# MengRao/pollnet

Hardware: AMD Instinct MI355X
Metric: device-resident Gbit/s + Mframes/s, 1500 B IPv4/TCP frames, 1/2/4/8 MI355X (higher is better)
Workload: dtype u16/u32 integer (one's-complement sums)

## Files before the change

pollnet_amd/csrc/rx_service.hip:

```cpp
#include <algorithm>
#include <chrono>
#include <cstdlib>

#include "rx_classify.hpp"

namespace {
using pn_internal::hip_err;
using pn_internal::set_err;

struct alignas(64) SvcPost {
  uint32_t gen;
  uint32_t n;
  uint32_t fpw;
  uint32_t max_conn;
  const uint8_t* frames;
  pn_result* out;
  const pn_conn_entry* tbl;
  uint16_t* links;
  uint32_t mask;
  uint32_t n_entries;
  uint32_t check;
  uint32_t seq;
};
static_assert(sizeof(SvcPost) == 64, "one line per post");

constexpr uint32_t kDoneWords = 64;
constexpr uint32_t kCountWords = 64;
constexpr uint32_t kExitWord = 96;
constexpr uint32_t kWordsBytes = 512;
constexpr uint32_t kLatWaves = PN_SERVICE_WAVES;
static_assert(kLatWaves <= kDoneWords, "a latency-tier post completes through per-wave done words");
constexpr uint32_t kLatFrames = kLatWaves * kFramesPerWave;
constexpr uint32_t kNetLimitMs = 8000;
constexpr uint32_t kPostVerify = 1u << 30, kPostLinks = 1u << 29, kPostN = (1u << 21) - 1;
constexpr uint32_t kLinkFrames = PN_LINK_MAX_FRAMES, kLinkConns = PN_LINK_MAX_CONNS;
constexpr uint32_t kMailBytes = 4096;

struct alignas(64) SvcDev {
  uint32_t count[2][16];
};
constexpr uint32_t kExitFlag = 32;

#ifdef PN_SVC_TRACE
__device__ uint64_t* g_svc_trace = nullptr;
#define SVC_T(w, i)                                                       \
  do {                                                                    \
    if (lane == 0 && (w) < 64) g_svc_trace[(w) * 8 + (i)] = wall_clock64(); \
  } while (0)
#else
#define SVC_T(w, i) \
  do {              \
  } while (0)
#endif

struct SArgs {
  const SvcPost* mail;
  u32x4* scratch;
  uint32_t* done_words;
  uint32_t* exit_word;
  SvcDev* dev;
  uint64_t idle_ticks;
  uint64_t net_ticks;
  uint32_t epoch;
  uint32_t last;
  uint32_t stride, ipa_off, avail;
  uint32_t poll_sleep;
};

inline uint32_t svc_fpw(uint32_t n, bool verify) {
  uint32_t fpw = verify ? 8u : kFramesPerWave;
  while (fpw < kFramesPerWave && (n + fpw - 1) / fpw > kLatWaves) fpw <<= 1;
  return fpw;
}

inline uint32_t svc_check(const SvcPost* p, uint32_t k) {
  const uint32_t* w = reinterpret_cast<const uint32_t*>(p);
  uint32_t x = k;
  for (int i = 1; i <= 13; i++) x ^= w[i];
  return x;
}

__host__ __device__ __forceinline__ uint32_t svc_active(uint32_t n, uint32_t fpw, uint32_t waves) {
  const uint32_t groups = (n + fpw - 1) / fpw;
  return groups < waves ? groups : waves;
}

inline uint32_t svc_helpers(uint32_t n, uint32_t max) {
  if (n <= kLatFrames) return 0;
  const uint32_t groups = (n + kFramesPerWave - 1) / kFramesPerWave;
  return std::min(groups - kLatWaves, max);
}

__device__ __forceinline__ KArgsAux svc_args(uint32_t v, uint32_t b, const SArgs& s, uint32_t k) {
  auto w32 = [&](uint32_t i) { return (uint32_t)__builtin_amdgcn_readlane(v, b + i); };
  auto u64 = [&](uint32_t lo) { return ((uint64_t)w32(lo + 1) << 32) | w32(lo); };
  KArgsAux a;
  const uint32_t nw = w32(1);
  a.n = nw & kPostN;
  a.fpw = w32(2) & 0xffu;
  a.max_conn = w32(3);
  a.frames = reinterpret_cast<const uint8_t*>(u64(4));
  a.out = reinterpret_cast<pn_result*>(u64(6));
  a.tbl = reinterpret_cast<const pn_conn_entry*>(u64(8));
  a.mask = w32(12);
  a.n_entries = w32(13);
  a.stride = s.stride;
  a.ipa_off = s.ipa_off;
  a.avail = s.avail;
  a.offs = nullptr;
  a.aux = (nw & kPostLinks) ? s.scratch + (size_t)(k & 1) * kLinkFrames * 2 : nullptr;
  return a;
}

__device__ __forceinline__ uint16_t* svc_links(uint32_t v, uint32_t b) {
  return reinterpret_cast<uint16_t*>(((uint64_t)(uint32_t)__builtin_amdgcn_readlane(v, b + 11) << 32) |
                                     (uint32_t)__builtin_amdgcn_readlane(v, b + 10));
}

constexpr uint32_t kCleanNeed = PN_F_HIT | PN_F_ACK | PN_F_IP_OK;
constexpr uint32_t kCleanNone = PN_F_TW | PN_F_SYN | PN_F_FIN | PN_F_RST | PN_F_NOT_TCP | PN_F_TRUNC | PN_F_BADOFF |
                                PN_F_IHL_NE_5;

struct ChainLds {
  uint32_t last[kLinkConns];
  uint32_t key[kLinkFrames];
  uint32_t seq_end[kLinkFrames];
  u32x4 fields[kLinkFrames];
};

__device__ __forceinline__ ChainLds& chain_lds() {
  __shared__ ChainLds c;
  return c;
}

__device__ __forceinline__ void chain_init(int lane) {
  ChainLds& c = chain_lds();
  for (uint32_t i = lane; i < kLinkConns; i += kWave) c.last[i] = 0u;
  wave_lds_sync();
}

__device__ __forceinline__ void chain_step(ChainLds& c, uint32_t base, uint32_t n, uint32_t max_conn, bool on,
                                           const u32x4& rec, const u32x4& fx, const __amdgpu_buffer_rsrc_t& lr,
                                           uint64_t below, int lane) {
  const uint32_t i = base + lane;
  const bool valid = i < n;
  const uint32_t flags = rec.w & 0xffffu;
  const uint32_t len = rec.z >> 16;
  const bool member = on && valid && (flags & (PN_F_HIT | PN_F_TW)) == PN_F_HIT && rec.x < max_conn;
  const bool usable = (flags & kCleanNeed) == kCleanNeed && (flags & kCleanNone) == 0 &&
                      (flags & (PN_F_TCP_OK | PN_F_TCP_UNCHECKED)) != 0 && len != 0 && len < 0x8000u;
  const uint32_t key = member ? rec.x : 0u;
  if (valid) {
    c.key[i] = member ? key : 0xFFFFFFFFu;
    c.seq_end[i] = rec.y + len;
    c.fields[i] = u32x4{fx.x, fx.y, fx.z, (rec.z & 0xffffu) | (usable ? 0x10000u : 0u)};
  }
  uint32_t prev = 0;
  if (member) prev = c.last[key];
  wave_lds_sync();
  if (member) atomicMax(&c.last[key], i + 1);
  wave_lds_sync();
  uint64_t todo = __ballot(member && c.last[key] != i + 1);
  while (todo) {
    const uint32_t leader = (uint32_t)__builtin_ctzll(todo);
    const uint32_t kk = __builtin_amdgcn_readlane(key, leader);
    const uint64_t m = __ballot(member && key == kk);
    todo &= ~m;
    const uint64_t lower = m & below;
    if (member && key == kk && lower) prev = base + 64u - (uint32_t)__builtin_clzll(lower);
  }
  uint32_t d = 0;
  if (member && usable && prev) {
    const uint32_t j = prev - 1;
    const u32x4 pf = c.fields[j];
    if ((pf.w >> 16) && c.seq_end[j] == rec.y && pf.x == fx.x && pf.y == fx.y && pf.z == fx.z &&
        (pf.w & 0xffffu) == (rec.z & 0xffffu))
      d = i - j;
  }
  if (valid) __builtin_amdgcn_raw_buffer_store_b16((unsigned short)d, lr, i * 2, 0, 0);
  wave_lds_sync();
}

__device__ __forceinline__ void chain_pass(const u32x4* aux, uint32_t n, uint32_t max_conn, uint16_t* links, int lane) {
  constexpr int kChunk = 8;
  ChainLds& c = chain_lds();
  const bool on = max_conn <= kLinkConns;
  const __amdgpu_buffer_rsrc_t lr = frame_rsrc(reinterpret_cast<const uint8_t*>(links), n * 2);
  const __amdgpu_buffer_rsrc_t ar = frame_rsrc(reinterpret_cast<const uint8_t*>(aux), n * 32);
  const uint64_t below = (1ull << lane) - 1;
  for (uint32_t base0 = 0; base0 < n; base0 += kChunk * kWave) {
    u32x4 rec[kChunk], fx[kChunk];
#pragma unroll
    for (int s = 0; s < kChunk; ++s) {
      const uint32_t i = base0 + s * kWave + lane;
      rec[s] = __builtin_amdgcn_raw_buffer_load_b128(ar, i * 32, 0, 0);
      fx[s] = __builtin_amdgcn_raw_buffer_load_b128(ar, i * 32 + 16, 0, 0);
    }
#pragma unroll
    for (int s = 0; s < kChunk; ++s)
      if (base0 + s * kWave < n) chain_step(c, base0 + s * kWave, n, max_conn, on, rec[s], fx[s], lr, below, lane);
  }
  for (uint32_t i = lane; i < n; i += kWave) {
    const uint32_t k = c.key[i];
    if (k != 0xFFFFFFFFu) c.last[k] = 0u;
  }
  wave_lds_sync();
}

template <int MIS, int COOP, bool HELPER = false>
__device__ __forceinline__ void svc_run(const KArgsAux& a, bool verify, bool linked, uint32_t w, uint32_t act, uint32_t k,
                                        uint32_t* done_word, int lane) {
  for (uint32_t g = w; g * a.fpw < a.n; g += act) {
    if (verify) classify_group<MIS, COOP, kProdAbl | kChainAux, kLoadAux, kStoreAux, 0, kLoadAux>(a, g * a.fpw, lane);
    else
      classify_group<MIS, COOP, kProdAbl | kHeaderOnly | kChainAux, kLoadAux, kStoreAux, 0, kLoadAux>(a, g * a.fpw, lane);
  }
  if constexpr (HELPER) return;
  __threadfence_system();
  if (lane == 0 && act <= kDoneWords && !linked)
    __hip_atomic_store(done_word, k, __ATOMIC_RELAXED, __HIP_MEMORY_SCOPE_SYSTEM);
}

template <bool PASS>
__device__ __forceinline__ void svc_finish(const KArgsAux& a, uint16_t* links, uint32_t k, uint32_t* count_word, int lane) {
  if constexpr (PASS) {
    if (a.aux) {
      __builtin_amdgcn_fence(__ATOMIC_ACQUIRE, "agent");
      chain_pass(a.aux, a.n, a.max_conn, links, lane);
    }
  }
  __threadfence_system();
  if (lane == 0) __hip_atomic_store(count_word, k, __ATOMIC_RELAXED, __HIP_MEMORY_SCOPE_SYSTEM);
}

template <bool PASS>
__device__ __forceinline__ void svc_count(uint32_t* count, const KArgsAux& a, uint16_t* links, uint32_t target, uint32_t k,
                                          uint32_t* count_word, int lane) {
  uint32_t prev = 0;
  if (lane == 0) prev = atomicAdd(count, 1u);
  prev = __builtin_amdgcn_readfirstlane(prev);
  if (prev == target - 1) {
    if (lane == 0) __hip_atomic_store(count, 0u, __ATOMIC_RELAXED, __HIP_MEMORY_SCOPE_AGENT);
    svc_finish<PASS>(a, links, k, count_word, lane);
  }
}

template <int MIS, int COOP>
__global__ __launch_bounds__(kWave) void rx_service_kernel(SArgs s) {
  const int lane = threadIdx.x;
  const uint32_t w = blockIdx.x, W = gridDim.x;
  const uint32_t* mw = reinterpret_cast<const uint32_t*>(s.mail);
  uint32_t last = s.last;
  uint64_t t0 = wall_clock64();
  chain_init(lane);
  for (;;) {
    const uint32_t v = lane <= (int)kExitFlag ? __hip_atomic_load(mw + lane, __ATOMIC_RELAXED, __HIP_MEMORY_SCOPE_SYSTEM) : 0u;
    if (w != 0 && (uint32_t)__builtin_amdgcn_readlane(v, kExitFlag) == s.epoch) return;
    const uint32_t k = last + 1;
    const uint32_t b = (k & 1) * 16;
    const uint32_t q = __builtin_amdgcn_readlane(v, b + 15);
    uint32_t x = q;
#pragma unroll
    for (uint32_t i = 1; i <= 13; i++) x ^= (uint32_t)__builtin_amdgcn_readlane(v, b + i);
    const bool whole = (uint32_t)__builtin_amdgcn_readlane(v, b) == q && (uint32_t)__builtin_amdgcn_readlane(v, b + 14) == x;
    if (!whole || (int32_t)(q - k) < 0) {
      if (w == 0) {
        if (wall_clock64() - t0 > s.idle_ticks) {
          if (lane == 0) {
            __hip_atomic_store(const_cast<uint32_t*>(mw) + kExitFlag, s.epoch, __ATOMIC_RELAXED, __HIP_MEMORY_SCOPE_SYSTEM);
            __hip_atomic_store(s.exit_word, s.epoch, __ATOMIC_RELEASE, __HIP_MEMORY_SCOPE_SYSTEM);
          }
          return;
        }
        __builtin_amdgcn_s_sleep(1);
      } else {
        if (wall_clock64() - t0 > s.net_ticks) return;
        for (uint32_t i = 0; i < s.poll_sleep; ++i) __builtin_amdgcn_s_sleep(1);
      }
      continue;
    }
    if (q != k) {
      last = k;
      t0 = wall_clock64();
      continue;
    }
    const uint32_t nw = __builtin_amdgcn_readlane(v, b + 1);
    if (nw == PN_SERVICE_STOP) return;
    last = k;
    const uint32_t fw = __builtin_amdgcn_readlane(v, b + 2);
    const uint32_t act = svc_active(nw & kPostN, fw & 0xffu, W + (fw >> 8));
    if (w < act) {
      SVC_T(w, 0);
      __builtin_amdgcn_fence(__ATOMIC_ACQUIRE, "");
      SVC_T(w, 1);
      const KArgsAux a = svc_args(v, b, s, k);
      SVC_T(w, 5);
      const bool linked = a.aux != nullptr;
      svc_run<MIS, COOP>(a, (nw & kPostVerify) != 0, linked, w, act, k, s.done_words + w, lane);
      SVC_T(w, 6);
      if (act > kDoneWords || linked) {
        uint32_t* cw = s.done_words + kCountWords + (k & 1);
        if (act == 1) svc_finish<true>(a, svc_links(v, b), k, cw, lane);
        else svc_count<true>(&s.dev->count[k & 1][0], a, svc_links(v, b), act < W ? act : W, k, cw, lane);
      }
      SVC_T(w, 7);
    }
    t0 = wall_clock64();
  }
}

template <int MIS, int COOP>
__global__ __launch_bounds__(kWave) void rx_service_helper_kernel(KArgsAux a, uint32_t verify, uint32_t act) {
  svc_run<MIS, COOP, true>(a, verify != 0, false, kLatWaves + blockIdx.x, act, 0, nullptr, threadIdx.x);
}

template <int MIS>
void launch_svc(bool coop, uint32_t waves, const SArgs& a, hipStream_t s) {
  if (coop) hipLaunchKernelGGL((rx_service_kernel<MIS, 1>), dim3(waves), dim3(kWave), 0, s, a);
  else hipLaunchKernelGGL((rx_service_kernel<MIS, 0>), dim3(waves), dim3(kWave), 0, s, a);
}

template <int MIS>
void launch_helpers(bool coop, uint32_t helpers, const KArgsAux& a, uint32_t verify, uint32_t act, hipStream_t s) {
  if (coop) hipLaunchKernelGGL((rx_service_helper_kernel<MIS, 1>), dim3(helpers), dim3(kWave), 0, s, a, verify, act);
  else hipLaunchKernelGGL((rx_service_helper_kernel<MIS, 0>), dim3(helpers), dim3(kWave), 0, s, a, verify, act);
}
}

struct pn_service {
  pn_ctx* ctx = nullptr;
  hipStream_t stream = nullptr;
  hipStream_t helper_stream = nullptr;
  uint32_t stride = 0, frame_off = 0;
  uint32_t helpers_max = 0;
  uint32_t post_helpers[2] = {0, 0};
  hipEvent_t helper_ev[2] = {nullptr, nullptr};
  uint64_t idle_ticks = 0, net_ticks = 0;
  SvcPost* mail = nullptr;
  bool mail_dev = false;
  uint32_t* words = nullptr;
  uint32_t post_words[2] = {0, 0};
  uint32_t tbl_post[2] = {0, 0};
  bool tbl_used[2] = {false, false};
  SvcDev* dev = nullptr;
  u32x4* scratch = nullptr;
  uint32_t seq = 0;
  uint32_t epoch = 0;
  bool running = false;
  bool coop = false;
};

namespace {
SArgs svc_sargs(const pn_service* v, uint32_t base) {
  SArgs a;
  a.mail = v->mail;
  a.scratch = v->scratch;
  a.done_words = v->words;
  a.exit_word = v->words + kExitWord;
  a.dev = v->dev;
  a.idle_ticks = v->idle_ticks;
  a.net_ticks = v->net_ticks;
  a.epoch = v->epoch;
  a.last = base;
  a.stride = v->stride;
  a.ipa_off = (v->frame_off + 14) & ~15u;
  a.avail = v->stride - v->frame_off;
  a.poll_sleep = v->mail_dev ? 1u : 16u;
  return a;
}

inline void host_sfence() { asm volatile("sfence" ::: "memory"); }

void svc_publish(SvcPost* slot, const SvcPost& q, bool wc) {
  static const bool avx = __builtin_cpu_supports("avx");
  if (wc && avx) {
    asm volatile(
        "vmovdqu (%0), %%ymm0\n\t"
        "vmovdqu 32(%0), %%ymm1\n\t"
        "vmovntdq %%ymm0, (%1)\n\t"
        "vmovntdq %%ymm1, 32(%1)\n\t"
        "sfence\n\t"
        "vzeroupper"
        :
        : "r"(&q), "r"(slot)
        : "memory", "xmm0", "xmm1");
    return;
  }
  volatile uint32_t* d = reinterpret_cast<volatile uint32_t*>(slot);
  const uint32_t* w = reinterpret_cast<const uint32_t*>(&q);
  for (int i = 1; i <= 14; ++i) d[i] = w[i];
  host_sfence();
  d[0] = w[0];
  d[15] = w[15];
  host_sfence();
}

int svc_launch_helpers(pn_service* v, uint32_t k, uint32_t helpers, const SvcPost& q) {
  KArgsAux a;
  strided_kargs(a, q.frames, q.out, q.tbl, q.mask, q.n_entries, q.max_conn, q.n & kPostN, v->stride, v->frame_off);
  a.fpw = q.fpw & 0xffu;
  const uint32_t verify = (q.n & kPostVerify) ? 1u : 0u, act = svc_active(a.n, a.fpw, kLatWaves + helpers);
  hipStream_t s = v->helper_stream;
  for_mis(v->frame_off, [&](auto mis) { launch_helpers<mis()>(v->coop, helpers, a, verify, act, s); });
  hipError_t e = hipGetLastError();
  if (e == hipSuccess && !v->helper_ev[k & 1]) e = hipEventCreateWithFlags(&v->helper_ev[k & 1], hipEventDisableTiming);
  if (e == hipSuccess) e = hipEventRecord(v->helper_ev[k & 1], s);
  if (e != hipSuccess) return hip_err(v->ctx, e, "pn_service: helper launch");
  return PN_OK;
}

int svc_launch(pn_service* v, uint32_t base) {
  pn_ctx* ctx = v->ctx;
  const SvcDev init{};
  hipError_t e = hipMemcpyAsync(v->dev, &init, sizeof(SvcDev), hipMemcpyHostToDevice, v->stream);
  if (e == hipSuccess) e = hipStreamSynchronize(v->stream);
  if (e != hipSuccess) return hip_err(ctx, e, "pn_service: device state");
  if (++v->epoch == 0) ++v->epoch;
  const SArgs a = svc_sargs(v, base);
  for_mis(v->frame_off, [&](auto mis) { launch_svc<mis()>(v->coop, kLatWaves, a, v->stream); });
  e = hipGetLastError();
  if (e != hipSuccess) return hip_err(ctx, e, "pn_service: launch");
  v->running = true;
  return PN_OK;
}

bool svc_post_ran(const pn_service* v, uint32_t k) {
  const uint32_t words = v->post_words[k & 1];
  if (words == 0 && (int32_t)(__atomic_load_n(v->words + kCountWords + (k & 1), __ATOMIC_ACQUIRE) - k) < 0) return false;
  for (uint32_t w = 0; w < words; ++w)
    if ((int32_t)(__atomic_load_n(v->words + w, __ATOMIC_ACQUIRE) - k) < 0) return false;
  if (v->post_helpers[k & 1] && hipEventQuery(v->helper_ev[k & 1]) != hipSuccess) return false;
  return true;
}

bool svc_post_done(const pn_service* v, uint32_t k) {
  if ((int32_t)(v->seq - k) >= 2) return true;
  if (!svc_post_ran(v, k)) return false;
  return k != v->seq || svc_post_ran(v, k - 1);
}

uint32_t svc_done(const pn_service* v) {
  if (svc_post_done(v, v->seq)) return v->seq;
  return svc_post_done(v, v->seq - 1) ? v->seq - 1 : v->seq - 2;
}

bool svc_exited(const pn_service* v) { return __atomic_load_n(v->words + kExitWord, __ATOMIC_ACQUIRE) == v->epoch; }

void svc_free(pn_service* v) {
  if (v->ctx) {
    auto& l = v->ctx->services;
    l.erase(std::remove(l.begin(), l.end(), v), l.end());
  }
  if (v->mail) (void)(v->mail_dev ? hipFree(v->mail) : hipHostFree(v->mail));
  if (v->words) (void)hipHostFree(v->words);
  if (v->dev) (void)hipFree(v->dev);
  if (v->scratch) (void)hipFree(v->scratch);
  if (v->stream) (void)hipStreamDestroy(v->stream);
  if (v->helper_stream) (void)hipStreamDestroy(v->helper_stream);
  for (hipEvent_t ev : v->helper_ev)
    if (ev) (void)hipEventDestroy(ev);
  delete v;
}
}

int pn_internal::svc_release_table(pn_ctx* ctx, int buf) {
  for (pn_service* v : ctx->services) {
    if (!v->tbl_used[buf]) continue;
    const uint32_t id = v->tbl_post[buf];
    if ((int32_t)(v->seq - id) < 2 && !svc_post_done(v, id)) {
      const int rc = pn_service_wait(v, id);
      if (rc) return rc;
    }
    v->tbl_used[buf] = false;
  }
  return PN_OK;
}

extern "C" {

int pn_service_open(pn_ctx* ctx, uint32_t slot_stride, uint32_t frame_off, uint32_t idle_ms, pn_service** out) {
  return pn_service_open_ex(ctx, slot_stride, frame_off, idle_ms, 0, out);
}

int pn_service_open_ex(pn_ctx* ctx, uint32_t slot_stride, uint32_t frame_off, uint32_t idle_ms, uint32_t large_waves,
                       pn_service** out) {
  if (!ctx || !out) return set_err(ctx, PN_EINVAL, "pn_service_open: ctx / out is NULL");
  *out = nullptr;
  if ((slot_stride & 15) || slot_stride > 65536 || (frame_off & 1) || slot_stride < frame_off + 96)
    return set_err(ctx, PN_EINVAL, "pn_service_open: slot_stride/frame_off violate the layout contract");
  if (idle_ms == 0 || idle_ms > 10000) return set_err(ctx, PN_EINVAL, "pn_service_open: idle_ms must be in [1, 10000]");
  if (large_waves && (large_waves < PN_SERVICE_WAVES || large_waves > PN_SERVICE_MAX_WAVES))
    return set_err(ctx, PN_EINVAL, "pn_service_open: large_waves must be 0 or in [PN_SERVICE_WAVES, PN_SERVICE_MAX_WAVES]");
  hipError_t e = hipSetDevice(ctx->device);
  if (e != hipSuccess) return hip_err(ctx, e, "hipSetDevice");
  int khz = 0;
  e = hipDeviceGetAttribute(&khz, hipDeviceAttributeWallClockRate, ctx->device);
  if (e != hipSuccess || khz <= 0) return hip_err(ctx, e, "pn_service_open: wall clock rate");
  int cus = 0;
  e = hipDeviceGetAttribute(&cus, hipDeviceAttributeMultiprocessorCount, ctx->device);
  if (e != hipSuccess || cus <= 0) return hip_err(ctx, e, "pn_service_open: CU count");
  pn_service* v = new pn_service();
  v->ctx = ctx;
  v->stride = slot_stride;
  v->frame_off = frame_off;
  const uint32_t total = large_waves ? large_waves
                                     : std::max<uint32_t>(kLatWaves, std::min<uint32_t>(PN_SERVICE_MAX_WAVES,
                                                                                      (uint32_t)cus * PN_SERVICE_WAVES_PER_CU));
  v->helpers_max = total - kLatWaves;
  v->idle_ticks = (uint64_t)khz * idle_ms;
  v->net_ticks = v->idle_ticks + (v->idle_ticks >> 1) + (uint64_t)khz * kNetLimitMs;
  v->coop = (slot_stride % 16) == 0 && ((frame_off + 14) & ~15u) >= 16;
  int large_bar = 0;
  if (hipDeviceGetAttribute(&large_bar, hipDeviceAttributeIsLargeBar, ctx->device) != hipSuccess) large_bar = 0;
  v->mail_dev = large_bar != 0 && std::getenv("PN_SERVICE_HOST_MAILBOX") == nullptr;
  if (v->mail_dev && hipExtMallocWithFlags((void**)&v->mail, kMailBytes, hipDeviceMallocUncached) != hipSuccess) {
    (void)hipGetLastError();
    v->mail = nullptr;
    v->mail_dev = false;
  }
  if ((e = hipStreamCreateWithFlags(&v->stream, hipStreamNonBlocking)) != hipSuccess ||
      (e = hipStreamCreateWithFlags(&v->helper_stream, hipStreamNonBlocking)) != hipSuccess ||
      (!v->mail && (e = hipHostMalloc((void**)&v->mail, kMailBytes, hipHostMallocDefault)) != hipSuccess) ||
      (e = hipHostMalloc((void**)&v->words, kWordsBytes, hipHostMallocDefault)) != hipSuccess ||
      (e = hipMalloc((void**)&v->dev, sizeof(SvcDev))) != hipSuccess ||
      (e = hipMalloc((void**)&v->scratch, sizeof(u32x4) * 2 * 2 * kLinkFrames)) != hipSuccess) {
    const int rc = hip_err(ctx, e, "pn_service_open: allocation");
    svc_free(v);
    return rc;
  }
  uint32_t first = 0;
  if (const char* env = std::getenv("PN_SERVICE_FIRST_POST")) first = (uint32_t)std::strtoull(env, nullptr, 0);
  std::memset(v->words, 0, kWordsBytes);
  for (uint32_t w = 0; w < kDoneWords + 2; ++w) v->words[w] = first;
  {
    SvcPost q{};
    q.gen = q.seq = first;
    q.check = ~svc_check(&q, first);
    for (int i = 0; i < 2; ++i) svc_publish(v->mail + i, q, v->mail_dev);
    volatile uint32_t* flag = reinterpret_cast<volatile uint32_t*>(v->mail) + kExitFlag;
    *flag = 0u;
    host_sfence();
  }
  v->seq = first;
  const int rc = svc_launch(v, first);
  if (rc) {
    svc_free(v);
    return rc;
  }
  ctx->services.push_back(v);
  *out = v;
  return PN_OK;
}

int pn_service_post(pn_service* v, const void* frames, uint32_t n, void* results, uint32_t* post_id) {
  return pn_service_post_linked(v, frames, n, results, nullptr, post_id);
}

int pn_service_post_linked(pn_service* v, const void* frames, uint32_t n, void* results, uint16_t* links,
                           uint32_t* post_id) {
  if (!v) return set_err(nullptr, PN_EINVAL, "pn_service_post: service is NULL");
  pn_ctx* ctx = v->ctx;
  if (!ctx->tbl_dev) return set_err(ctx, PN_ENOTABLE, "pn_service_post: no conn table (call pn_set_conn_table)");
  if (n == 0 || n > PN_SERVICE_MAX_FRAMES || !frames || !results)
    return set_err(ctx, PN_EINVAL, "pn_service_post: n must be in [1, PN_SERVICE_MAX_FRAMES], buffers set");
  if (((uintptr_t)frames & 15) || ((uintptr_t)results & 15))
    return set_err(ctx, PN_EINVAL, "pn_service_post: frames/results must be 16-byte aligned");
  if (links && (n > PN_LINK_MAX_FRAMES || ((uintptr_t)links & 1)))
    return set_err(ctx, PN_EINVAL, "pn_service_post_linked: n must be <= PN_LINK_MAX_FRAMES, links 2-byte aligned");
  const uint32_t done = svc_done(v);
  if ((int32_t)(v->seq - done) >= 2) return set_err(ctx, PN_EINVAL, "pn_service_post: two posts already outstanding");
  if (v->running && svc_exited(v)) v->running = false;
  if (!v->running) {
    const int rc = svc_launch(v, done);
    if (rc) return rc;
  }
  const uint32_t k = v->seq + 1;
  const bool verify = ctx->verify_tcp;
  SvcPost q{};
  q.n = n | (verify ? kPostVerify : 0u) | (links ? kPostLinks : 0u);
  q.max_conn = ctx->max_conn;
  q.frames = (const uint8_t*)frames;
  q.out = (pn_result*)results;
  q.tbl = ctx->tbl_dev;
  q.links = links;
  q.mask = (uint32_t)ctx->mask;
  q.n_entries = ctx->n_entries;
  const uint32_t fpw = svc_fpw(n, verify), helpers = svc_helpers(n, v->helpers_max);
  q.fpw = fpw | helpers << 8;
  const uint32_t act = svc_active(n, fpw, kLatWaves + helpers);
  if (helpers) {
    const int rc = svc_launch_helpers(v, k, helpers, q);
    if (rc) return rc;
  }
  v->post_helpers[k & 1] = helpers;
  v->post_words[k & 1] = (act <= kDoneWords && !links) ? act : 0u;
  v->tbl_post[ctx->cur] = k;
  v->tbl_used[ctx->cur] = true;
  q.check = svc_check(&q, k);
  q.gen = q.seq = k;
  svc_publish(v->mail + (k & 1), q, v->mail_dev);
  v->seq = k;
  if (post_id) *post_id = k;
  return PN_OK;
}

int pn_service_wait(pn_service* v, uint32_t post_id) {
  if (!v) return set_err(nullptr, PN_EINVAL, "pn_service_wait: service is NULL");
  if (post_id == 0 || (int32_t)(post_id - v->seq) > 0 || (int32_t)(v->seq - post_id) >= 2)
    post_id = v->seq;
  const uint32_t k = post_id;
  const auto t_start = std::chrono::steady_clock::now();
  for (uint64_t i = 1;; ++i) {
    if (svc_post_done(v, k)) return PN_OK;
    if ((i & 4095) == 0) {
      if (std::chrono::steady_clock::now() - t_start > std::chrono::seconds(10))
        return set_err(v->ctx, PN_EHIP, "pn_service_wait: no completion within 10 s");
      if (svc_exited(v)) {
        const uint32_t done = svc_done(v);
        if ((int32_t)(done - k) >= 0) return PN_OK;
        v->running = false;
        const int rc = svc_launch(v, done);
        if (rc) return rc;
        continue;
      }
      const hipError_t q = hipStreamQuery(v->stream);
      if (q != hipErrorNotReady && q != hipSuccess) return hip_err(v->ctx, q, "pn_service_wait: the service kernel failed");
      if (q == hipSuccess && !svc_post_done(v, k) && !svc_exited(v))
        return set_err(v->ctx, PN_EHIP, "pn_service_wait: the service kernel ended without completing the post");
    }
  }
}

int pn_service_close(pn_service* v) {
  if (!v) return PN_OK;
  pn_ctx* ctx = v->ctx;
  int rc = svc_post_done(v, v->seq) ? PN_OK : pn_service_wait(v, 0);
  if (v->running && !svc_exited(v)) {
    const uint32_t k = v->seq + 1;
    SvcPost q{};
    q.n = PN_SERVICE_STOP;
    v->post_words[k & 1] = 0;
    v->post_helpers[k & 1] = 0;
    q.check = svc_check(&q, k);
    q.gen = q.seq = k;
    svc_publish(v->mail + (k & 1), q, v->mail_dev);
    v->seq = k;
  }
  hipError_t e = hipStreamSynchronize(v->stream);
  if (e == hipSuccess) e = hipStreamSynchronize(v->helper_stream);
  if (e != hipSuccess && rc == PN_OK) rc = hip_err(ctx, e, "pn_service_close");
  svc_free(v);
  return rc;
}

}

#ifdef PN_SVC_TRACE
extern "C" int pn_svc_trace_set(uint64_t* host_buf) {
  return hipMemcpyToSymbol(HIP_SYMBOL(g_svc_trace), &host_buf, sizeof host_buf) == hipSuccess ? PN_OK : PN_EHIP;
}
#endif
```

Before: 52460.

## Size helper grid to one wave per frame group with dedicated lean helper kernel

The helper kernel now takes plain KArgs without the aux chain path, drops the trailing system fence, maps blocks across XCDs, and sets launch bounds for occupancy 4. The helper grid cap is no longer derived from CU count times waves-per-CU but from the maximum number of frame groups, so large posts can launch one wave per group instead of looping. Helper launch failures are now recorded and surfaced in wait. This trades more launched waves and scheduling overhead for less per-wave looping and lower register pressure.

```diff
diff --git a/pollnet_amd/csrc/rx_service.hip b/pollnet_amd/csrc/rx_service.hip
--- a/pollnet_amd/csrc/rx_service.hip
+++ b/pollnet_amd/csrc/rx_service.hip
@@ -33,6 +33,8 @@
 constexpr uint32_t kLatFrames = kLatWaves * kFramesPerWave;
 constexpr uint32_t kNetLimitMs = 8000;
 constexpr uint32_t kPostVerify = 1u << 30, kPostLinks = 1u << 29, kPostN = (1u << 21) - 1;
+constexpr uint32_t kMaxGroups = kPostN / kFramesPerWave + 1;
+static_assert(PN_SERVICE_MAX_FRAMES <= kPostN && kMaxGroups < (1u << 24), "the n and fpw words hold every post");
 constexpr uint32_t kLinkFrames = PN_LINK_MAX_FRAMES, kLinkConns = PN_LINK_MAX_CONNS;
 constexpr uint32_t kMailBytes = 4096;
 
@@ -207,7 +209,7 @@
   wave_lds_sync();
 }
 
-template <int MIS, int COOP, bool HELPER = false>
+template <int MIS, int COOP>
 __device__ __forceinline__ void svc_run(const KArgsAux& a, bool verify, bool linked, uint32_t w, uint32_t act, uint32_t k,
                                         uint32_t* done_word, int lane) {
   for (uint32_t g = w; g * a.fpw < a.n; g += act) {
@@ -215,7 +217,6 @@
     else
       classify_group<MIS, COOP, kProdAbl | kHeaderOnly | kChainAux, kLoadAux, kStoreAux, 0, kLoadAux>(a, g * a.fpw, lane);
   }
-  if constexpr (HELPER) return;
   __threadfence_system();
   if (lane == 0 && act <= kDoneWords && !linked)
     __hip_atomic_store(done_word, k, __ATOMIC_RELAXED, __HIP_MEMORY_SCOPE_SYSTEM);
@@ -310,8 +311,14 @@
 }
 
 template <int MIS, int COOP>
-__global__ __launch_bounds__(kWave) void rx_service_helper_kernel(KArgsAux a, uint32_t verify, uint32_t act) {
-  svc_run<MIS, COOP, true>(a, verify != 0, false, kLatWaves + blockIdx.x, act, 0, nullptr, threadIdx.x);
+__global__ __launch_bounds__(kWave, 4) void rx_service_helper_kernel(KArgs a, uint32_t verify, uint32_t act) {
+  for (uint32_t g = kLatWaves + xcd_group(blockIdx.x, gridDim.x); g * a.fpw < a.n; g += act) {
+    int l = threadIdx.x;
+    asm volatile("" : "+v"(l));
+    const int lane = l & (kWave - 1);
+    if (verify) classify_group<MIS, COOP, kProdAbl, kLoadAux, kStoreAux, 0, kLoadAux>(a, g * a.fpw, lane);
+    else classify_group<MIS, COOP, kProdAbl | kHeaderOnly, kLoadAux, kStoreAux, 0, kLoadAux>(a, g * a.fpw, lane);
+  }
 }
 
 template <int MIS>
@@ -321,7 +328,7 @@
 }
 
 template <int MIS>
-void launch_helpers(bool coop, uint32_t helpers, const KArgsAux& a, uint32_t verify, uint32_t act, hipStream_t s) {
+void launch_helpers(bool coop, uint32_t helpers, const KArgs& a, uint32_t verify, uint32_t act, hipStream_t s) {
   if (coop) hipLaunchKernelGGL((rx_service_helper_kernel<MIS, 1>), dim3(helpers), dim3(kWave), 0, s, a, verify, act);
   else hipLaunchKernelGGL((rx_service_helper_kernel<MIS, 0>), dim3(helpers), dim3(kWave), 0, s, a, verify, act);
 }
@@ -335,6 +342,7 @@
   uint32_t helpers_max = 0;
   uint32_t post_helpers[2] = {0, 0};
   hipEvent_t helper_ev[2] = {nullptr, nullptr};
+  mutable hipError_t helper_err = hipSuccess;
   uint64_t idle_ticks = 0, net_ticks = 0;
   SvcPost* mail = nullptr;
   bool mail_dev = false;
@@ -396,7 +404,7 @@
 }
 
 int svc_launch_helpers(pn_service* v, uint32_t k, uint32_t helpers, const SvcPost& q) {
-  KArgsAux a;
+  KArgs a;
   strided_kargs(a, q.frames, q.out, q.tbl, q.mask, q.n_entries, q.max_conn, q.n & kPostN, v->stride, v->frame_off);
   a.fpw = q.fpw & 0xffu;
   const uint32_t verify = (q.n & kPostVerify) ? 1u : 0u, act = svc_active(a.n, a.fpw, kLatWaves + helpers);
@@ -429,7 +437,13 @@
   if (words == 0 && (int32_t)(__atomic_load_n(v->words + kCountWords + (k & 1), __ATOMIC_ACQUIRE) - k) < 0) return false;
   for (uint32_t w = 0; w < words; ++w)
     if ((int32_t)(__atomic_load_n(v->words + w, __ATOMIC_ACQUIRE) - k) < 0) return false;
-  if (v->post_helpers[k & 1] && hipEventQuery(v->helper_ev[k & 1]) != hipSuccess) return false;
+  if (v->post_helpers[k & 1]) {
+    const hipError_t e = hipEventQuery(v->helper_ev[k & 1]);
+    if (e != hipSuccess) {
+      if (e != hipErrorNotReady) v->helper_err = e;
+      return false;
+    }
+  }
   return true;
 }
 
@@ -496,17 +510,11 @@
   int khz = 0;
   e = hipDeviceGetAttribute(&khz, hipDeviceAttributeWallClockRate, ctx->device);
   if (e != hipSuccess || khz <= 0) return hip_err(ctx, e, "pn_service_open: wall clock rate");
-  int cus = 0;
-  e = hipDeviceGetAttribute(&cus, hipDeviceAttributeMultiprocessorCount, ctx->device);
-  if (e != hipSuccess || cus <= 0) return hip_err(ctx, e, "pn_service_open: CU count");
   pn_service* v = new pn_service();
   v->ctx = ctx;
   v->stride = slot_stride;
   v->frame_off = frame_off;
-  const uint32_t total = large_waves ? large_waves
-                                     : std::max<uint32_t>(kLatWaves, std::min<uint32_t>(PN_SERVICE_MAX_WAVES,
-                                                                                      (uint32_t)cus * PN_SERVICE_WAVES_PER_CU));
-  v->helpers_max = total - kLatWaves;
+  v->helpers_max = large_waves ? large_waves - kLatWaves : kMaxGroups - kLatWaves;
   v->idle_ticks = (uint64_t)khz * idle_ms;
   v->net_ticks = v->idle_ticks + (v->idle_ticks >> 1) + (uint64_t)khz * kNetLimitMs;
   v->coop = (slot_stride % 16) == 0 && ((frame_off + 14) & ~15u) >= 16;
@@ -612,6 +620,7 @@
   const auto t_start = std::chrono::steady_clock::now();
   for (uint64_t i = 1;; ++i) {
     if (svc_post_done(v, k)) return PN_OK;
+    if (v->helper_err != hipSuccess) return hip_err(v->ctx, v->helper_err, "pn_service_wait: the helper grid failed");
     if ((i & 4095) == 0) {
       if (std::chrono::steady_clock::now() - t_start > std::chrono::seconds(10))
         return set_err(v->ctx, PN_EHIP, "pn_service_wait: no completion within 10 s");
```

Result: no change. 52360 (-0.2%).
